# qq456cvb/SLAM-MaskRCNN

Hardware: AMD Instinct MI355X
Metric: Mvoxel-updates/s + frames/s, 512^3 semantic TSDF @ 640x480 (higher is better)
Workload: dtype f32; 1 GPU; C3: 512^3 semantic TSDF integrate (sdf f32, weight i32, colour u8x3, 32-bin u32 instance histogram), synthetic 640x480 depth+RGB+mask stream (seed 1, noise on), frames resident in HBM; frames_cycled=16

## Files before the change

### include/semtsdf.h

```cpp
#ifndef SEMTSDF_H
#define SEMTSDF_H

#include <stddef.h>
#include <stdint.h>

#ifdef __cplusplus
extern "C" {
#endif

#define SEMTSDF_ABI_VERSION 12
#define SEMTSDF_MAX_OBJECTS 32

#define SEMTSDF_OK 0
#define SEMTSDF_ERR_INVALID (-1)
#define SEMTSDF_ERR_HIP (-2)
#define SEMTSDF_ERR_OOM (-3)
#define SEMTSDF_ERR_LABEL (-4)
#define SEMTSDF_ERR_STATE (-5)
#define SEMTSDF_ERR_COMM (-6)
#define SEMTSDF_ERR_UNSUPPORTED (-7)
#define SEMTSDF_NEED_PIXELS 1

#define SEMTSDF_F_SEMANTIC 0x1u
#define SEMTSDF_F_GATE_COLOR 0x2u
// ... 182 lines not shown
typedef struct semtsdf_instance {
    uint64_t voxels;
    uint64_t votes;
    uint64_t support;
    uint64_t sum[3];
    uint64_t rgb_sum[3];
    uint32_t min[3], max[3];
} semtsdf_instance;
int semtsdf_instance_stats(semtsdf_vol* v, float sdf_max, int32_t min_weight,
                           semtsdf_instance out[SEMTSDF_MAX_OBJECTS], uint64_t* overlap );
int semtsdf_remap_instances(semtsdf_vol* v, const uint8_t lut[SEMTSDF_MAX_OBJECTS], int32_t num_objs,
                            void* stream);

int semtsdf_map_words(semtsdf_vol* v, uint64_t* out, uint64_t capacity, uint64_t* count);

int semtsdf_set_instrumentation(semtsdf_vol* v, int enable);
int semtsdf_get_timing(semtsdf_vol* v, semtsdf_timing* out);
int semtsdf_reset_timing(semtsdf_vol* v);

int semtsdf_tsdf_update(float* tsdf_diff, int32_t* tsdf_color, int32_t* tsdf_wt, int32_t* tsdf_cls,
                        int32_t* tsdf_cls_cnt, int vol_dim, const float* vol_start, float voxel,
                        float miu, const float* intrinsic, const uint16_t* depth, const uint8_t* color,
                        const int32_t* cls, const float* extrinsic2init, int width, int height);

#ifdef __cplusplus
}
#endif
#endif
```

### slam-maskrcnn_amd/csrc/semtsdf_api.cpp

```cpp
#include <hip/hip_runtime.h>

#include <algorithm>
#include <cmath>
#include <cstdarg>
#include <cstdio>
#include <cstdlib>
#include <cstring>
#include <mutex>
#include <string>
#include <vector>

#include "../../include/semtsdf.h"
#include "semtsdf_internal.h"

using namespace semtsdf;

namespace {

thread_local std::string g_err;

int fail(int code, const char* fmt, ...) {
    char buf[1024];
    va_list ap;
    va_start(ap, fmt);
// ... 68 lines not shown
    uint8_t* palette_d = nullptr;
    uint8_t* render_d = nullptr;
    float* render_t_d = nullptr;
    unsigned long long* counters_d = nullptr;
    IntegrateRare* rare_d = nullptr;
    float* rcp_table_d = nullptr;
    AssocDecision* decision_h = nullptr;
    void* ray_state_d = nullptr;
    MarchCamera ray_cam{};
    int ray_kind = -1;
    int ray_nrec = 1;
    int ray_next = 0;
    uint32_t n_obs = 0;
    bool maps_dirty = false;
    bool maps_stale = true;
    hipEvent_t maps_ev = nullptr;
    bool maps_ev_set = false;
    hipStream_t map_stream = nullptr;
    bool map_set = false;
    bool multi_stream = false;
    bool color_wide = false;
    int64_t wmax_bound = 0;
    const uint8_t* pending_lut = nullptr;
    unsigned long long* wtrace_d = nullptr;
    unsigned* tile_cost_d = nullptr;
    unsigned* tile_perm_d = nullptr;
    int tile_cap = 0, tile_n = 0;
    bool tables_clean = false;
    unsigned long long votes_dropped_seen = 0;
    int instr = 0;
// ... 9 lines not shown
size_t npx(const semtsdf_vol* v) { return (size_t)v->p.width * (size_t)v->p.height; }

hipStream_t pick(const semtsdf_vol* v, void* s) { return s ? (hipStream_t)s : v->stream; }

int dev_alloc(semtsdf_vol* v, void** p, size_t bytes) {
    if (bytes == 0) { *p = nullptr; return SEMTSDF_OK; }
    hipError_t e = hipMalloc(p, bytes);
    if (e != hipSuccess)
        return fail(e == hipErrorOutOfMemory ? SEMTSDF_ERR_OOM : SEMTSDF_ERR_HIP, "hipMalloc(%zu): %s", bytes,
                    hipGetErrorString(e));
    v->device_bytes += bytes;
    return SEMTSDF_OK;
}

void free_all(semtsdf_vol* v) {
    void* ptrs[] = {v->b.sdf, v->b.wt, v->b.bplain, v->b.boct, v->b.botmp, v->b.bdirty, v->b.dlist, v->b.sflag, v->b.color, v->b.hist, v->b.hmask, v->b.cls, v->b.cls_cnt, v->depth_d, v->rgb_d,
                    v->mask_d, v->cls_d, v->tables_d, v->decision_d,
                    v->num_objs_d, v->probs_d, v->box_d, v->palette_d, v->render_d, v->render_t_d,
                    v->counters_d, v->ray_state_d, v->rcp_table_d, v->wtrace_d, v->exact_d, v->px.bits, v->px.p, v->tile_cost_d, v->tile_perm_d, v->rare_d};
    for (void* q : ptrs)
        if (q) (void)hipFree(q);
    for (auto& f : v->fs)
        for (void* q : {(void*)f.pyr.px, (void*)f.pyr.l0, (void*)f.pyr.l1, (void*)f.unit_list, (void*)f.list_count,
                        (void*)f.units})
            if (q) (void)hipFree(q);
    if (v->decision_h) (void)hipHostFree(v->decision_h);
    for (auto* vec : {&v->ev_integrate, &v->ev_assoc, &v->ev_render, &v->ev_prep})
        for (auto& e : *vec) { (void)hipEventDestroy(e.a); (void)hipEventDestroy(e.b); }
    if (v->maps_ev) (void)hipEventDestroy(v->maps_ev);
    for (auto& f : v->fs) {
        if (f.prep_done) (void)hipEventDestroy(f.prep_done);
// ... 254 lines not shown
            fwrite(h.data(), 8, h.size(), f);
            fclose(f);
        }
    }
    if (ep.a) v->ev_integrate.push_back(ep);
    F.reader = s;
    if (v->async_used && async && own_order) {
        F.free_recorded = false;
    } else if (v->async_used || s != v->stream) {
        if (!F.set_free)
            if (int rc = ensure_prep_stream(v)) return rc;
        HIPC(hipEventRecord(F.set_free, s));
        F.free_recorded = true;
    }
    v->maps_dirty = true;
    v->n_integrate++;
    return SEMTSDF_OK;
}

MarchCamera assoc_camera(const semtsdf_vol* v, const float E[16]) {
    MarchCamera c{};
    const float* Ki = v->p.Kinv;
    c.Kinv[0] = Ki[0]; c.Kinv[1] = Ki[1]; c.Kinv[2] = Ki[2];
    c.Kinv[3] = Ki[4]; c.Kinv[4] = Ki[5]; c.Kinv[5] = Ki[6];
    c.Kinv[6] = Ki[8]; c.Kinv[7] = Ki[9]; c.Kinv[8] = Ki[10];
    for (int i = 0; i < 3; ++i)
        for (int j = 0; j < 3; ++j) c.Rt[i * 3 + j] = E[j * 4 + i];
    for (int i = 0; i < 3; ++i) {
        const double acc = (double)c.Rt[i * 3 + 0] * (double)E[3] + (double)c.Rt[i * 3 + 1] * (double)E[7] +
                           (double)c.Rt[i * 3 + 2] * (double)E[11];
// ... 3 lines not shown
    return c;
}

int order_after_map(semtsdf_vol* v, hipStream_t s) {
    if (!v->map_set || v->map_stream == s) return SEMTSDF_OK;
    v->multi_stream = true;
    if (!v->maps_ev_set) {
        if (!v->maps_ev) HIPC(hipEventCreateWithFlags(&v->maps_ev, order_event_flags()));
        HIPC(hipEventRecord(v->maps_ev, v->map_stream));
        v->maps_ev_set = true;
    }
    HIPC(hipStreamWaitEvent(s, v->maps_ev, 0));
    return SEMTSDF_OK;
}

int ensure_maps(semtsdf_vol* v, hipStream_t s) {
    if (int rc = order_after_map(v, s)) return rc;
    if (!v->maps_dirty && !v->maps_stale) return SEMTSDF_OK;
    HIPC(launch_brick_min(v->g, v->b, v->maps_stale, s));
    v->map_stream = s;
    v->map_set = true;
    v->maps_ev_set = false;
    if (v->multi_stream || s != v->stream) {
        if (!v->maps_ev) HIPC(hipEventCreateWithFlags(&v->maps_ev, order_event_flags()));
        HIPC(hipEventRecord(v->maps_ev, s));
        v->maps_ev_set = true;
    }
    v->maps_dirty = false;
    v->maps_stale = false;
    return SEMTSDF_OK;
}

int after_maps(semtsdf_vol* v, hipStream_t s) { return order_after_map(v, s); }

// ... 350 lines not shown
    const size_t n = g.nvox;
    const size_t px = (size_t)p->width * p->height;
    auto bail = [&](int code) { free_all(v); delete v; return code; };
    int prio_least = 0, prio_greatest = 0;
    if (hipDeviceGetStreamPriorityRange(&prio_least, &prio_greatest) != hipSuccess) prio_greatest = 0;
    if (hipStreamCreateWithPriority(&v->stream, hipStreamNonBlocking, prio_greatest) != hipSuccess)
        return bail(fail(SEMTSDF_ERR_HIP, "hipStreamCreate failed"));
    const bool ci32 = p->flags & SEMTSDF_F_COLOR_I32;
    if ((rc = dev_alloc(v, (void**)&v->b.sdf, n * 4))) return bail(rc);
    if ((rc = dev_alloc(v, (void**)&v->b.wt, n * 4))) return bail(rc);
    if ((rc = dev_alloc(v, (void**)&v->b.sflag, n / 32 + 1))) return bail(rc);
    const size_t nbricks = (size_t)g.nbx * g.nby * g.nbz;
    if ((rc = dev_alloc(v, (void**)&v->b.bplain, nbricks * 4))) return bail(rc);
    if ((rc = dev_alloc(v, (void**)&v->b.boct, nbricks * 8))) return bail(rc);
    if ((rc = dev_alloc(v, (void**)&v->b.botmp, nbricks * 8))) return bail(rc);
    const size_t nquads = (size_t)g.nbx * g.nby * (size_t)((g.nbz + 3) / 4);
    if ((rc = dev_alloc(v, (void**)&v->b.bdirty, nquads * 4))) return bail(rc);
    if ((rc = dev_alloc(v, (void**)&v->b.dlist, (nquads + 1) * 4))) return bail(rc);
    if (nquads && (hipMemset(v->b.bdirty, 0, nquads * 4) != hipSuccess || hipMemset(v->b.dlist, 0, 4) != hipSuccess))
        return bail(fail(SEMTSDF_ERR_HIP, "memset failed"));
    (void)ci32;
    if ((rc = dev_alloc(v, &v->b.color, g.nvox * 4))) return bail(rc);
    if (p->flags & SEMTSDF_F_SEMANTIC)
    {
        if ((rc = dev_alloc(v, (void**)&v->b.hist, g.nvox * kMaxObjects * 4))) return bail(rc);
        if ((rc = dev_alloc(v, (void**)&v->b.hmask, n * 4))) return bail(rc);
    }
    if (p->flags & SEMTSDF_F_VOTE) {
        if ((rc = dev_alloc(v, (void**)&v->b.cls, n * 4))) return bail(rc);
        if ((rc = dev_alloc(v, (void**)&v->b.cls_cnt, n * 4))) return bail(rc);
// ... 964 lines not shown
    }
    v->maps_stale = true;
    HIPC(hipStreamSynchronize(s));
    return SEMTSDF_OK;
}

int semtsdf_map_words(semtsdf_vol* v, uint64_t* out, uint64_t capacity, uint64_t* count) {
    if (!v || !count) return fail(SEMTSDF_ERR_INVALID, "NULL argument");
    HIPC(hipSetDevice(v->device));
    hipStream_t s = v->stream;
    *count = (uint64_t)v->g.nbx * v->g.nby * v->g.nbz;
    if (int rc = ensure_maps(v, s)) return rc;
    const uint64_t n = std::min<uint64_t>(capacity, *count);
    if (out && n) HIPC(hipMemcpyAsync(out, v->b.boct, n * sizeof(uint64_t), hipMemcpyDeviceToHost, s));
    HIPC(hipStreamSynchronize(s));
    return SEMTSDF_OK;
}

int semtsdf_export_surface(semtsdf_vol* v, float sdf_max, int32_t min_weight, semtsdf_surface_point* out,
                           uint64_t capacity, uint64_t* count) {
    static_assert(sizeof(semtsdf_surface_point) == sizeof(SurfacePoint), "surface point layout");
    if (!v || !count) return fail(SEMTSDF_ERR_INVALID, "NULL argument");
    if (!(sdf_max > 0.0f)) return fail(SEMTSDF_ERR_INVALID, "sdf_max must be > 0");
    HIPC(hipSetDevice(v->device));
    hipStream_t s = v->stream;
    if (int rc = after_maps(v, s)) return rc;
    unsigned long long* cnt_d = nullptr;
    HIPC(hipMalloc((void**)&cnt_d, sizeof(unsigned long long)));
    SurfacePoint* pts_d = nullptr;
    auto cleanup = [&]() {
// ... 299 lines not shown
```

### slam-maskrcnn_amd/csrc/semtsdf_internal.h

```cpp
#pragma once
#include <hip/hip_runtime_api.h>
#include <stdint.h>

namespace semtsdf {

constexpr int kMaxObjects = 32;
constexpr int kMaxDetections = 256;
constexpr int kRcpTable = 1024;
constexpr int kZAlign = 32;
#ifndef SEMTSDF_BRICK_DIST_CAP
#define SEMTSDF_BRICK_DIST_CAP 16
#endif
constexpr int kBrickDistCap = SEMTSDF_BRICK_DIST_CAP;
constexpr int kListSegs = 64;
constexpr unsigned kPreWaves = 65534;
constexpr unsigned kFirstTabSlots = kListSegs * 256;
constexpr int kListCountStride = 64;
constexpr int kLists = 3;
constexpr int kListTotalsWord = kLists * kListSegs * kListCountStride;
constexpr int kListCountWords = kListTotalsWord + 8;

struct VolGeom {
    int dimx, dimy, dimz;
    int lz;
// ... 22 lines not shown
struct VolBufs {
    float* sdf;
    int32_t* wt;
    void* color;
    uint32_t* hist;
    uint32_t* hmask;
    int32_t* cls;
    int32_t* cls_cnt;
    float* bplain;
    uint64_t* boct;
    uint64_t* botmp;
    uint32_t* bdirty;
    uint32_t* dlist;
    uint8_t* sflag;
};

struct DepthPyramid {
    uint2* px;
    uint2* l0;
    uint2* l1;
    int w0, h0, w1, h1;
    unsigned rs;
};

__device__ inline unsigned rec_index(const DepthPyramid& p, unsigned u, unsigned v) {
    return __umul24(v >> 2, p.rs) + ((u << 2) | (v & 3u));
}

struct IntegrateRare {
    uint32_t* bdirty;
// ... 174 lines not shown
hipError_t launch_shard_ray_step(const ShardRayArgs& a, hipStream_t s);
hipError_t launch_shard_render_final(const ShardRayArgs& a, hipStream_t s);
hipError_t launch_shard_render_finish(const ShardRayArgs& a, hipStream_t s);
hipError_t launch_shard_assoc_partial(const ShardRayArgs& a, hipStream_t s);
hipError_t launch_shard_assoc_pixels(const ShardRayArgs& a, int32_t* out, hipStream_t s);
hipError_t launch_tables_from_partial(const long long* reduced, AssocTables* t, hipStream_t s);
hipError_t launch_copy_f4(const void* src, void* dst, size_t n16, hipStream_t s);
hipError_t launch_min_i64(long long* dst, const long long* src, size_t n, hipStream_t s);
hipError_t launch_masks_to_labels(const uint8_t* masks, int npx, int n, int min_area, void* scratch, uint8_t* out,
                                  hipStream_t s);
size_t mask_scratch_bytes();
size_t mask_scratch_kept_offset();
hipError_t launch_detections_to_labels(const int32_t* boxes, const void* mini, int dtype, int mh, int mw, int n,
                                       int width, int height, int min_area, void* scratch, uint8_t* out,
                                       uint32_t* areas, hipStream_t s);
hipError_t launch_brick_min(const VolGeom& g, const VolBufs& b, bool all, hipStream_t s);
hipError_t launch_fill_volume(const VolGeom& g, const VolBufs& b, uint32_t flags, hipStream_t s);
hipError_t launch_depth_pyramid(const uint16_t* depth, const uint8_t* rgb, uint8_t* mask, int w, int h,
                                float scale, const DepthPyramid& p, unsigned* list_count, hipStream_t s,
                                const uint8_t* lut = nullptr);
hipError_t launch_vox_chunk(const void* src, void* dst, bool to_ref, const VolGeom& g, uint64_t v0, uint64_t nv,
                            hipStream_t s);
hipError_t launch_color_widen(const uint8_t* narrow, int32_t* wide, uint64_t nvox, hipStream_t s);
hipError_t launch_color_chunk(const void* src, void* dst, bool to_ref, bool ref_i32, bool dev_i32, const VolGeom& g,
                              uint64_t v0, uint64_t nv, hipStream_t s);
hipError_t launch_integrate(const IntegrateArgs& a, hipStream_t s, hipEvent_t e0 = nullptr,
                            hipEvent_t e1 = nullptr);
uint64_t unit_count(const VolGeom& g);
uint64_t unit_list_capacity(const VolGeom& g);
int unit_grid_fits(int dimx, int dimy, int local_z);
hipError_t launch_cull(const IntegrateArgs& a, hipStream_t s);
// ... 62 lines not shown
```

### slam-maskrcnn_amd/csrc/semtsdf_kernels.hip

```cpp
#include <hip/hip_runtime.h>
#include <hip/hip_ext.h>
#include <stdint.h>
#include <limits.h>
#include <stddef.h>
#include <stdlib.h>
#include "semtsdf_internal.h"
#include "semtsdf_libm.h"
#include "semtsdf_steps.h"

namespace semtsdf {

__device__ __forceinline__ int f2i_rd(float x) {
    const float f = floorf(x);
    if (!(f == f)) return 0;
    if (f >= 2147483648.0f) return INT_MAX;
    if (f <= -2147483648.0f) return INT_MIN;
    return (int)f;
}

__device__ __forceinline__ float dot3(float a0, float a1, float a2, float b0, float b1, float b2) {
    return fmaf(a2, b2, fmaf(a1, b1, a0 * b0));
}

typedef float f32x2 __attribute__((ext_vector_type(2)));
// ... 99 lines not shown
}

__global__ __launch_bounds__(256) void k_min_i64(long long* __restrict__ dst, const long long* __restrict__ src, size_t n) {
    for (size_t i = (size_t)blockIdx.x * blockDim.x + threadIdx.x; i < n; i += (size_t)gridDim.x * blockDim.x)
        dst[i] = min(dst[i], src[i]);
}

hipError_t launch_min_i64(long long* dst, const long long* src, size_t n, hipStream_t s) {
    size_t blocks = (n + 255) / 256;
    if (blocks > 4096) blocks = 4096;
    if (blocks == 0) return hipSuccess;
    hipLaunchKernelGGL(k_min_i64, dim3((unsigned)blocks), dim3(256), 0, s, dst, src, n);
    return hipGetLastError();
}

__device__ __forceinline__ void brick_quad_min(const VolGeom& g, const float* __restrict__ sdf,
                                               float* __restrict__ plain, unsigned q, unsigned want) {
    const unsigned nbq = (unsigned)(g.nbz + 3) / 4;
    const int lane = threadIdx.x & 63;
    const int bq = q % nbq, by = (q / nbq) % g.nby, bx = q / (nbq * g.nby);
    const unsigned br0 = ((unsigned)bx * g.nby + (unsigned)by) * g.nbz + (unsigned)bq * 4;
    const int nbr = min(4, g.nbz - bq * 4);
    const int x = bx * 8 + (lane >> 3), y = by * 8 + (lane & 7), z0 = bq * 32;
    float m[4] = {3.0e38f, 3.0e38f, 3.0e38f, 3.0e38f};
    if (x < g.dimx && y < g.dimy) {
        const float* p = sdf + tile_index(g, x, y, z0);
        if (z0 + 32 <= g.lz) {
#pragma unroll
            for (int j = 0; j < 4; ++j) {
                const float4 a = *reinterpret_cast<const float4*>(p + 64 * j);
                const float4 c = *reinterpret_cast<const float4*>(p + 64 * j + 32);
                m[j] = fminf(fminf(fminf(a.x, a.y), fminf(a.z, a.w)), fminf(fminf(c.x, c.y), fminf(c.z, c.w)));
            }
        } else {
            for (int k = 0; k < g.lz - z0; ++k) {
                const float v = p[tile_zterm(k)];
#pragma unroll
                for (int j = 0; j < 4; ++j) m[j] = (k >> 3) == j ? fminf(m[j], v) : m[j];
            }
        }
    }
#pragma unroll
    for (int j = 0; j < 4; ++j)
        for (int off = 32; off > 0; off >>= 1) m[j] = fminf(m[j], __shfl_xor(m[j], off, 64));
    if (lane < nbr && ((want >> lane) & 1u)) {
        const float mj = lane == 0 ? m[0] : lane == 1 ? m[1] : lane == 2 ? m[2] : m[3];
        plain[br0 + lane] = mj;
    }
}

__global__ __launch_bounds__(256) void k_brick_plain(VolGeom g, const float* __restrict__ sdf, float* __restrict__ plain,
                                                     uint32_t* __restrict__ dirty, const uint32_t* __restrict__ dlist,
                                                     int all) {
    const unsigned nbq = (unsigned)(g.nbz + 3) / 4;
    const unsigned nq = (unsigned)g.nbx * g.nby * nbq;
    const unsigned w0 = blockIdx.x * 4 + (threadIdx.x >> 6);
    if (all) {
        if (w0 >= nq) return;
        brick_quad_min(g, sdf, plain, w0, 0xFu);
        if ((threadIdx.x & 63) == 0) dirty[w0] = 0u;
        return;
    }
    const unsigned n = dlist[0];
    for (unsigned i = w0; i < n; i += gridDim.x * 4) {
        const unsigned q = dlist[1 + i];
        const unsigned want = dirty[q];
        brick_quad_min(g, sdf, plain, q, want);
        if ((threadIdx.x & 63) == 0) dirty[q] = 0u;
    }
}

__device__ __forceinline__ float skip_threshold(const VolGeom& g);

__global__ __launch_bounds__(256) void k_brick_dilate(VolGeom g, const float* __restrict__ plain,
                                                      uint64_t* __restrict__ d0, uint32_t* __restrict__ dlist) {
    const unsigned nb = (unsigned)g.nbx * g.nby * g.nbz;
    const unsigned br = blockIdx.x * blockDim.x + threadIdx.x;
    if (br == 0) dlist[0] = 0u;
    if (br >= nb) return;
    const int bz = br % g.nbz, by = (br / g.nbz) % g.nby, bx = br / (g.nbz * g.nby);
    float m = 3.0e38f;
    for (int i = 0; i < 2; ++i)
        for (int j = 0; j < 2; ++j)
            for (int k = 0; k < 2; ++k) {
                const int xx = bx + i, yy = by + j, zz = bz + k;
                if (xx < g.nbx && yy < g.nby && zz < g.nbz) m = fminf(m, plain[((unsigned)xx * g.nby + yy) * g.nbz + zz]);
            }
    d0[br] = m >= skip_threshold(g) ? (uint64_t)kBrickDistCap * 0x0101010101010101ull : 0ull;
}

typedef unsigned short u16x2 __attribute__((ext_vector_type(2)));

template <int AXIS>
__device__ __forceinline__ void oct_unpack(uint64_t wp, uint64_t wn, u16x2 R[4]) {
    const uint32_t pl = (uint32_t)wp, ph = (uint32_t)(wp >> 32), nl = (uint32_t)wn, nh = (uint32_t)(wn >> 32);
    uint32_t r0, r1, r2, r3;
    if (AXIS == 0) {
        r0 = pl & 0x00FF00FFu; r1 = (nl >> 8) & 0x00FF00FFu;
        r2 = ph & 0x00FF00FFu; r3 = (nh >> 8) & 0x00FF00FFu;
    } else if (AXIS == 1) {
        r0 = (pl & 0x000000FFu) | (nl & 0x00FF0000u); r1 = ((pl >> 8) & 0x000000FFu) | ((nl >> 8) & 0x00FF0000u);
        r2 = (ph & 0x000000FFu) | (nh & 0x00FF0000u); r3 = ((ph >> 8) & 0x000000FFu) | ((nh >> 8) & 0x00FF0000u);
    } else {
        r0 = pl & 0x00FF00FFu; r1 = (pl >> 8) & 0x00FF00FFu;
        r2 = nh & 0x00FF00FFu; r3 = (nh >> 8) & 0x00FF00FFu;
    }
    R[0] = __builtin_bit_cast(u16x2, r0); R[1] = __builtin_bit_cast(u16x2, r1);
    R[2] = __builtin_bit_cast(u16x2, r2); R[3] = __builtin_bit_cast(u16x2, r3);
}

template <int AXIS>
__global__ __launch_bounds__(256) void k_brick_oct_axis(VolGeom g, const uint64_t* __restrict__ in,
                                                        uint64_t* __restrict__ out) {
    const unsigned nb = (unsigned)g.nbx * g.nby * g.nbz;
    const unsigned br = blockIdx.x * blockDim.x + threadIdx.x;
    if (br >= nb) return;
    const int bz = br % g.nbz, by = (br / g.nbz) % g.nby, bx = br / (g.nbz * g.nby);
    const int pos = AXIS == 0 ? bx : AXIS == 1 ? by : bz;
    const int n = AXIS == 0 ? g.nbx : AXIS == 1 ? g.nby : g.nbz;
    const int stride = AXIS == 0 ? g.nby * g.nbz : AXIS == 1 ? g.nbz : 1;
    const uint64_t v = in[br];
    u16x2 d[4];
    oct_unpack<0>(v, v, d);
    auto hmax = [](const u16x2* x) {
        const u16x2 m = __builtin_elementwise_max(__builtin_elementwise_max(x[0], x[1]),
                                                  __builtin_elementwise_max(x[2], x[3]));
        return (int)max(m.x, m.y);
    };
    int dmax = hmax(d);
    for (int k0 = 1; k0 < kBrickDistCap && k0 < dmax; k0 += 4) {
        uint64_t wp[4], wn[4];
// ... 3 lines not shown
            wp[i] = (k < kBrickDistCap && pos + k < n) ? in[(int)br + k * stride] : ~0ull;
            wn[i] = (k < kBrickDistCap && pos - k >= 0) ? in[(int)br - k * stride] : ~0ull;
        }
#pragma unroll
        for (int i = 0; i < 4; ++i) {
            u16x2 w[4];
            oct_unpack<AXIS>(wp[i], wn[i], w);
            const u16x2 kk = {(unsigned short)(k0 + i), (unsigned short)(k0 + i)};
#pragma unroll
            for (int j = 0; j < 4; ++j) d[j] = __builtin_elementwise_min(d[j], __builtin_elementwise_max(w[j], kk));
        }
        dmax = hmax(d);
    }
    const uint32_t lo = (uint32_t)d[0].x | ((uint32_t)d[1].x << 8) | ((uint32_t)d[0].y << 16) | ((uint32_t)d[1].y << 24);
    const uint32_t hi = (uint32_t)d[2].x | ((uint32_t)d[3].x << 8) | ((uint32_t)d[2].y << 16) | ((uint32_t)d[3].y << 24);
    out[br] = (uint64_t)lo | ((uint64_t)hi << 32);
}

hipError_t launch_brick_min(const VolGeom& g, const VolBufs& b, bool all, hipStream_t s) {
    const unsigned nb = (unsigned)g.nbx * g.nby * g.nbz;
    if (nb == 0) return hipSuccess;
    const unsigned nq = (unsigned)g.nbx * g.nby * (unsigned)((g.nbz + 3) / 4);
    const unsigned nw = all ? nq : (nq < 4096u ? nq : 4096u);
    hipLaunchKernelGGL(k_brick_plain, dim3((nw + 3) / 4), dim3(256), 0, s, g, b.sdf, b.bplain, b.bdirty, b.dlist,
                       all ? 1 : 0);
    hipLaunchKernelGGL(k_brick_dilate, dim3((nb + 255) / 256), dim3(256), 0, s, g, b.bplain, b.botmp, b.dlist);
    hipLaunchKernelGGL(k_brick_oct_axis<0>, dim3((nb + 255) / 256), dim3(256), 0, s, g, b.botmp, b.boct);
    hipLaunchKernelGGL(k_brick_oct_axis<1>, dim3((nb + 255) / 256), dim3(256), 0, s, g, b.boct, b.botmp);
    hipLaunchKernelGGL(k_brick_oct_axis<2>, dim3((nb + 255) / 256), dim3(256), 0, s, g, b.botmp, b.boct);
    return hipGetLastError();
}

hipError_t launch_fill_volume(const VolGeom& g, const VolBufs& b, uint32_t flags, hipStream_t s) {
    (void)flags;
    const uint64_t n = g.nvox;
    uint64_t blocks = (n / 4 + 255) / 256;
    if (blocks > 8192) blocks = 8192;
    if (blocks == 0) blocks = 1;
    hipLaunchKernelGGL(k_fill_f32, dim3((unsigned)blocks), dim3(256), 0, s, b.sdf, n, g.mu);
    return hipGetLastError();
}

__device__ __forceinline__ void pyramid_tile(const uint16_t* __restrict__ depth, const uint8_t* __restrict__ rgb,
                                             uint8_t* mask, int w, int h, float scale, int vec, const DepthPyramid& p,
// ... 888 lines not shown
template <bool SEM, bool CI32, bool VOTE, bool FREE>
__device__ __forceinline__ void stage_store(const IntegrateArgs& a, const UnitPos& up, unsigned coff,
                                            const StoreMeta& M, const Out& O) {
    const VolGeom& g = a.g;
    const unsigned tmask = M.meta & 15u, gmask = (M.meta >> 4) & 15u, hmode = (M.meta >> 8) & 3u,
                   hlab = M.meta >> 16;
    const bool line = ((__ballot(tmask != 0u) >> ((int)__lane_id() % LZQ + lane_slot((int)__lane_id()) * kUnitLanes)) &
                       kLineLanes) != 0ull;
    if (!line) return;
    const uint64_t v = O.ub + coff;
    {
        const uint64_t cb = __ballot(O.cross);
        const __attribute__((address_space(4))) IntegrateRare* R =
            (const __attribute__((address_space(4))) IntegrateRare*)a.rare;
        if (cb && R->bdirty) {
            const int lane = (int)__lane_id(), j = lane % kUnitLanes;
            const int bz = (up.uz * UZ >> 3) + j;
            const uint64_t pj = ((kLineLanes << (2 * (j & 3))) | (kLineLanes << (2 * (j & 3) + 1)))
                                << (lane_slot(lane) * kUnitLanes);
            if (j < UZ / 8 && (cb & pj) && bz < R->nbz) {
                const unsigned nbq = (unsigned)(R->nbz + 3) >> 2;
                const unsigned q = __umul24(__umul24((unsigned)(up.x * UX >> 3), (unsigned)R->nby) +
                                                (unsigned)(up.uy * UY >> 3), nbq) + ((unsigned)bz >> 2);
                __attribute__((address_space(1))) uint32_t* bd = (__attribute__((address_space(1))) uint32_t*)R->bdirty;
                __attribute__((address_space(1))) uint32_t* dl = (__attribute__((address_space(1))) uint32_t*)R->dlist;
                if (__hip_atomic_fetch_or(bd + q, 1u << (bz & 3), __ATOMIC_RELAXED, __HIP_MEMORY_SCOPE_AGENT) == 0u)
                    dl[1 + __hip_atomic_fetch_add(dl, 1u, __ATOMIC_RELAXED, __HIP_MEMORY_SCOPE_AGENT)] = q;
            }
        }
    }
    if (!(kProbes && a.debug == 10) && tmask != 0u) {
        if (!O.skip) st_state(a.b.sdf + v, O.s4);
        st_state(a.b.wt + v, O.w4);
    }
    {
// ... 2951 lines not shown
```

### slam-maskrcnn_amd/semtsdf/_lib.py

```python
from __future__ import annotations

import ctypes as C
import os

import numpy as np

_HERE = os.path.dirname(os.path.abspath(__file__))
LIB_PATH = os.path.join(_HERE, "libsemtsdf.so")

MAX_OBJECTS = 32

OK = 0
ERR_INVALID = -1
ERR_HIP = -2
ERR_OOM = -3
ERR_LABEL = -4
ERR_STATE = -5
ERR_COMM = -6
ERR_UNSUPPORTED = -7

F_SEMANTIC = 0x1
F_GATE_COLOR = 0x2
F_COLOR_I32 = 0x4
F_VOTE = 0x8
# ... 90 lines not shown
        ("n_integrate", C.c_uint64),
        ("n_assoc", C.c_uint64),
        ("n_render", C.c_uint64),
        ("touched", C.c_uint64),
        ("gated", C.c_uint64),
        ("bricks", C.c_uint64),
        ("prep_ms", C.c_double),
        ("n_prep", C.c_uint64),
        ("free_units", C.c_uint64),
        ("full_units", C.c_uint64),
        ("lazy_voxels", C.c_uint64),
        ("assoc_exact_frames", C.c_uint64),
        ("assoc_exact_rows", C.c_uint64),
        ("touched_lines", C.c_uint64),
        ("assoc_pos_max", C.c_double),
    ]


_P = C.c_void_p
_I = C.c_int
_F = C.c_float
_D = C.c_double
_PP = C.POINTER(C.c_void_p)

SIGNATURES = {
    "semtsdf_last_error": (C.c_char_p, []),
    "semtsdf_abi_version": (_I, []),
    "semtsdf_build_key": (C.c_char_p, []),
    "semtsdf_device_count": (_I, [C.POINTER(C.c_int)]),
    "semtsdf_set_device": (_I, [_I]),
# ... 38 lines not shown
    "semtsdf_shard_note_integrated": (_I, [_P, _P, _P]),
    "semtsdf_min_i64": (_I, [_P, _P, C.c_size_t, _P]),
    "semtsdf_masks_to_labels": (_I, [_P, _I, _I, _I, _I, _P, C.POINTER(C.c_int), _P]),
    "semtsdf_detections_to_labels_workspace": (C.c_size_t, [_I]),
    "semtsdf_detections_to_labels": (_I, [_P, _P, _I, _I, _I, _I, _I, _I, _I, _P, _P, _P, C.POINTER(C.c_int), _P]),
    "semtsdf_copy_bandwidth": (_I, [_I, C.c_size_t, _I, C.POINTER(C.c_double)]),
    "semtsdf_download": (_I, [_P, _P, _P, _P, _P, _P, _P]),
    "semtsdf_download_slab": (_I, [_P, _I, _I, _P, _P, _P, _P, _P, _P]),
    "semtsdf_upload": (_I, [_P, _P, _P, _P, _P, _P, _P]),
    "semtsdf_export_surface": (_I, [_P, _F, C.c_int32, _P, C.c_uint64, C.POINTER(C.c_uint64)]),
    "semtsdf_extract_mesh": (_I, [_P, C.c_int32, _P, C.c_uint64, _P, C.c_uint64, C.POINTER(C.c_uint64),
                                  C.POINTER(C.c_uint64)]),
    "semtsdf_instance_stats": (_I, [_P, _F, C.c_int32, _P, _P]),
    "semtsdf_remap_instances": (_I, [_P, _P, C.c_int32, _P]),
    "semtsdf_map_words": (_I, [_P, _P, C.c_uint64, C.POINTER(C.c_uint64)]),
    "semtsdf_set_instrumentation": (_I, [_P, _I]),
    "semtsdf_get_timing": (_I, [_P, C.POINTER(Timing)]),
    "semtsdf_reset_timing": (_I, [_P]),
    "semtsdf_tsdf_update": (_I, [_P, _P, _P, _P, _P, _I, _P, _F, _F, _P, _P, _P, _P, _P, _I, _I]),
}

_lib = None
_load_error = None


def _bind_torch_runtime():
    if os.environ.get("SEMTSDF_NO_TORCH") == "1":
        return
    try:
        import torch
# ... 53 lines not shown
```

### slam-maskrcnn_amd/semtsdf/volume.py

```python
from __future__ import annotations

import ctypes as C

import numpy as np

from . import _lib as L


def default_params(dim, intrinsics, width, height) -> L.Params:
    lib = L.load()
    p = L.Params()
    intr = L.f32(intrinsics, 4)
    L.check(lib.semtsdf_params_default(C.byref(p), int(dim), L.ptr(intr), int(width), int(height)))
    return p


def place_from_frame(p: L.Params, depth: np.ndarray, mean_depth: float, mode: int) -> L.Params:
    lib = L.load()
    d = np.ascontiguousarray(depth, dtype=np.uint16)
    if d.size != p.width * p.height:
        raise ValueError("depth size does not match params")
    L.check(lib.semtsdf_place_from_frame(C.byref(p), L.ptr(d), float(mean_depth), int(mode)))
    return p

# ... 230 lines not shown
                c(cls, np.int32), c(cls_cnt, np.int32)]
        L.check(L.load().semtsdf_upload(self._h, *[L.ptr(a) for a in arrs]))

    def instance_stats(self, sdf_max: float = 0.2, min_weight: int = 1, overlap: bool = True) -> dict:
        from .instances import instance_stats

        return instance_stats(self, sdf_max, min_weight, overlap)

    def remap_instances(self, lut, num_objs: int = -1, stream=None):
        t = np.ascontiguousarray(np.asarray(lut).reshape(-1))
        if t.size != L.MAX_OBJECTS or (t < 0).any() or (t > 255).any():
            raise ValueError(f"lut must hold {L.MAX_OBJECTS} ids")
        t = t.astype(np.uint8)
        L.check(L.load().semtsdf_remap_instances(self._h, L.ptr(t), int(num_objs), stream))

    def set_instrumentation(self, events: bool = True, count: bool = False, force_exact: bool = False):
        flags = (1 if events else 0) | (2 if count else 0) | (4 if force_exact else 0)
        L.check(L.load().semtsdf_set_instrumentation(self._h, flags))

    def map_words(self):
        import numpy as np
        n = C.c_uint64(0)
        L.check(L.load().semtsdf_map_words(self._h, None, 0, C.byref(n)))
        if n.value == 0:
            return None
        out = np.zeros(n.value, dtype=np.uint64)
        L.check(L.load().semtsdf_map_words(self._h, C.c_void_p(out.ctypes.data), n.value, C.byref(n)))
        return out

    def filter_overlaps_dev(self, probs_ptr: int, box_ptr: int, mask_ptr: int, stream=None) -> L.AssocStats:
        st = L.AssocStats()
        L.check(L.load().semtsdf_filter_overlaps_dev(self._h, C.c_void_p(probs_ptr), C.c_void_p(box_ptr),
                                                     C.c_void_p(mask_ptr), C.byref(st), stream))
        return st

    def timing(self) -> L.Timing:
        t = L.Timing()
        L.check(L.load().semtsdf_get_timing(self._h, C.byref(t)))
        return t

    def reset_timing(self):
        L.check(L.load().semtsdf_reset_timing(self._h))
```

Before: 1.652 million Mvoxel-updates/s.

## Add incremental brick distance-map update driven by flip lists

Adds an incremental mode for the brick skip map: the plain-min pass records bricks whose skip classification flips, then seed and per-axis octahedral distance passes recompute only neighbourhoods of changed bricks using epoch stamps and bounded lists, falling back to full passes on overflow. The aim is to avoid full-volume map rebuilds after each integrate. Separately, the integrate kernel's dirty-brick marking now elects a single lane per crossed brick to cut redundant atomic writes. Adds extra buffers, atomics and a stats API; incremental mode is gated by a brick-count threshold or env/flag.

```diff
diff --git a/include/semtsdf.h b/include/semtsdf.h
--- a/include/semtsdf.h
+++ b/include/semtsdf.h
@@ -220,6 +220,17 @@
 
 int semtsdf_map_words(semtsdf_vol* v, uint64_t* out, uint64_t capacity, uint64_t* count);
 
+typedef struct semtsdf_map_stats {
+    uint32_t incremental;
+    uint32_t dirty_quads;
+    uint32_t plain_flips;
+    uint32_t seed_flips;
+    uint32_t changed[3];
+    uint32_t overflow;
+    uint32_t capacity;
+} semtsdf_map_stats;
+int semtsdf_get_map_stats(semtsdf_vol* v, semtsdf_map_stats* out);
+
 int semtsdf_set_instrumentation(semtsdf_vol* v, int enable);
 int semtsdf_get_timing(semtsdf_vol* v, semtsdf_timing* out);
 int semtsdf_reset_timing(semtsdf_vol* v);
diff --git a/slam-maskrcnn_amd/csrc/semtsdf_api.cpp b/slam-maskrcnn_amd/csrc/semtsdf_api.cpp
--- a/slam-maskrcnn_amd/csrc/semtsdf_api.cpp
+++ b/slam-maskrcnn_amd/csrc/semtsdf_api.cpp
@@ -106,6 +106,10 @@
     uint32_t n_obs = 0;
     bool maps_dirty = false;
     bool maps_stale = true;
+    MapInc mi{};
+    int maps_pending = 0;
+    uint32_t map_epoch = 0;
+    uint32_t map_inc_epoch0 = 0;
     hipEvent_t maps_ev = nullptr;
     bool maps_ev_set = false;
     hipStream_t map_stream = nullptr;
@@ -145,7 +149,7 @@
 }
 
 void free_all(semtsdf_vol* v) {
-    void* ptrs[] = {v->b.sdf, v->b.wt, v->b.bplain, v->b.boct, v->b.botmp, v->b.bdirty, v->b.dlist, v->b.sflag, v->b.color, v->b.hist, v->b.hmask, v->b.cls, v->b.cls_cnt, v->depth_d, v->rgb_d,
+    void* ptrs[] = {v->b.sdf, v->b.wt, v->b.bplain, v->b.boct, v->b.botmp, v->mi.seed, v->mi.octx, v->mi.ctl, v->mi.lists, v->mi.stamp, v->b.bdirty, v->b.dlist, v->b.sflag, v->b.color, v->b.hist, v->b.hmask, v->b.cls, v->b.cls_cnt, v->depth_d, v->rgb_d,
                     v->mask_d, v->cls_d, v->tables_d, v->decision_d,
                     v->num_objs_d, v->probs_d, v->box_d, v->palette_d, v->render_d, v->render_t_d,
                     v->counters_d, v->ray_state_d, v->rcp_table_d, v->wtrace_d, v->exact_d, v->px.bits, v->px.p, v->tile_cost_d, v->tile_perm_d, v->rare_d};
@@ -430,6 +434,7 @@
         F.free_recorded = true;
     }
     v->maps_dirty = true;
+    v->maps_pending++;
     v->n_integrate++;
     return SEMTSDF_OK;
 }
@@ -463,10 +468,31 @@
     return SEMTSDF_OK;
 }
 
+bool maps_incremental(const semtsdf_vol* v) {
+    static const char* env = getenv("SEMTSDF_MAP_INCREMENTAL");
+    if (env && *env) return atoi(env) != 0;
+    if (v->instr & 8) return true;
+    return (uint64_t)v->g.nbx * v->g.nby * v->g.nbz >= kMapIncMinBricks;
+}
+
 int ensure_maps(semtsdf_vol* v, hipStream_t s) {
     if (int rc = order_after_map(v, s)) return rc;
     if (!v->maps_dirty && !v->maps_stale) return SEMTSDF_OK;
-    HIPC(launch_brick_min(v->g, v->b, v->maps_stale, s));
+    uint32_t epoch0 = 0;
+    const bool inc = !v->maps_stale && maps_incremental(v) && v->maps_pending <= kMapIncMaxFrames;
+    v->maps_pending = 0;
+    if (inc) {
+        if (v->map_epoch > 0xFFFFFFF0u) {
+            const size_t nb = (size_t)v->g.nbx * v->g.nby * v->g.nbz;
+            HIPC(hipMemsetAsync(v->mi.stamp, 0, nb * sizeof(uint32_t), s));
+            HIPC(hipMemsetAsync(v->mi.ctl + kMapOvf, 0, kMapLists * sizeof(uint32_t), s));
+            v->map_epoch = 0;
+        }
+        epoch0 = v->map_epoch + 1;
+        v->map_epoch += 4;
+    }
+    HIPC(launch_brick_min(v->g, v->b, v->mi, v->maps_stale ? kMapAll : inc ? kMapIncremental : kMapDirty, epoch0, s));
+    v->map_inc_epoch0 = epoch0;
     v->map_stream = s;
     v->map_set = true;
     v->maps_ev_set = false;
@@ -847,6 +873,15 @@
     if ((rc = dev_alloc(v, (void**)&v->b.bplain, nbricks * 4))) return bail(rc);
     if ((rc = dev_alloc(v, (void**)&v->b.boct, nbricks * 8))) return bail(rc);
     if ((rc = dev_alloc(v, (void**)&v->b.botmp, nbricks * 8))) return bail(rc);
+    if ((rc = dev_alloc(v, (void**)&v->mi.seed, nbricks * 8))) return bail(rc);
+    if ((rc = dev_alloc(v, (void**)&v->mi.octx, nbricks * 8))) return bail(rc);
+    v->mi.cap = map_list_capacity(nbricks);
+    if ((rc = dev_alloc(v, (void**)&v->mi.ctl, kMapCtlWords * 4))) return bail(rc);
+    if ((rc = dev_alloc(v, (void**)&v->mi.lists, (size_t)kMapLists * v->mi.cap * 4))) return bail(rc);
+    if ((rc = dev_alloc(v, (void**)&v->mi.stamp, nbricks * 4))) return bail(rc);
+    if (hipMemset(v->mi.ctl, 0, kMapCtlWords * 4) != hipSuccess ||
+        (nbricks && hipMemset(v->mi.stamp, 0, nbricks * 4) != hipSuccess))
+        return bail(fail(SEMTSDF_ERR_HIP, "memset failed"));
     const size_t nquads = (size_t)g.nbx * g.nby * (size_t)((g.nbz + 3) / 4);
     if ((rc = dev_alloc(v, (void**)&v->b.bdirty, nquads * 4))) return bail(rc);
     if ((rc = dev_alloc(v, (void**)&v->b.dlist, (nquads + 1) * 4))) return bail(rc);
@@ -1841,6 +1876,28 @@
     const uint64_t n = std::min<uint64_t>(capacity, *count);
     if (out && n) HIPC(hipMemcpyAsync(out, v->b.boct, n * sizeof(uint64_t), hipMemcpyDeviceToHost, s));
     HIPC(hipStreamSynchronize(s));
+    return SEMTSDF_OK;
+}
+
+int semtsdf_get_map_stats(semtsdf_vol* v, semtsdf_map_stats* out) {
+    if (!v || !out) return fail(SEMTSDF_ERR_INVALID, "NULL argument");
+    HIPC(hipSetDevice(v->device));
+    *out = semtsdf_map_stats{};
+    out->capacity = v->mi.cap;
+    if (!v->map_set) return SEMTSDF_OK;
+    uint32_t c[kMapCtlWords];
+    HIPC(hipDeviceSynchronize());
+    HIPC(hipMemcpy(c, v->mi.ctl, sizeof(c), hipMemcpyDeviceToHost));
+    if (!v->map_inc_epoch0) return SEMTSDF_OK;
+    out->incremental = 1;
+    out->dirty_quads = c[kMapStatQuads];
+    out->plain_flips = c[kMapStatPlain];
+    out->seed_flips = c[kMapStatSeed];
+    out->changed[0] = c[kMapStatX];
+    out->changed[1] = c[kMapCnt + kMapListXY];
+    out->changed[2] = c[kMapCnt + kMapListXYZ];
+    for (int i = 0; i < kMapLists; ++i)
+        if (c[kMapOvf + i] == v->map_inc_epoch0) out->overflow |= 1u << i;
     return SEMTSDF_OK;
 }
 
diff --git a/slam-maskrcnn_amd/csrc/semtsdf_internal.h b/slam-maskrcnn_amd/csrc/semtsdf_internal.h
--- a/slam-maskrcnn_amd/csrc/semtsdf_internal.h
+++ b/slam-maskrcnn_amd/csrc/semtsdf_internal.h
@@ -60,6 +60,36 @@
     uint32_t* dlist;
     uint8_t* sflag;
 };
+
+constexpr int kMapListPlain = 0;
+constexpr int kMapListSeed = 1;
+constexpr int kMapListX = 2;
+constexpr int kMapListXY = 3;
+constexpr int kMapListXYZ = 4;
+constexpr int kMapLists = 4;
+constexpr int kMapCnt = 0;
+constexpr int kMapOvf = 5;
+constexpr int kMapStatQuads = 9;
+constexpr int kMapStatPlain = 10;
+constexpr int kMapStatSeed = 11;
+constexpr int kMapStatX = 12;
+constexpr int kMapCtlWords = 16;
+constexpr unsigned kMapIncBlocks = 1024;
+constexpr int kMapAll = 0, kMapDirty = 1, kMapIncremental = 2;
+constexpr uint64_t kMapIncMinBricks = 1u << 20;
+constexpr int kMapIncMaxFrames = 4;
+struct MapInc {
+    uint64_t* seed;
+    uint64_t* octx;
+    uint32_t* ctl;
+    uint32_t* lists;
+    uint32_t* stamp;
+    unsigned cap;
+};
+inline unsigned map_list_capacity(uint64_t nbricks) {
+    const uint64_t c = nbricks / 32u;
+    return (unsigned)(c < 256u ? 256u : c);
+}
 
 struct DepthPyramid {
     uint2* px;
@@ -264,7 +294,8 @@
 hipError_t launch_detections_to_labels(const int32_t* boxes, const void* mini, int dtype, int mh, int mw, int n,
                                        int width, int height, int min_area, void* scratch, uint8_t* out,
                                        uint32_t* areas, hipStream_t s);
-hipError_t launch_brick_min(const VolGeom& g, const VolBufs& b, bool all, hipStream_t s);
+hipError_t launch_brick_min(const VolGeom& g, const VolBufs& b, const MapInc& m, int mode, uint32_t epoch0,
+                            hipStream_t s);
 hipError_t launch_fill_volume(const VolGeom& g, const VolBufs& b, uint32_t flags, hipStream_t s);
 hipError_t launch_depth_pyramid(const uint16_t* depth, const uint8_t* rgb, uint8_t* mask, int w, int h,
                                 float scale, const DepthPyramid& p, unsigned* list_count, hipStream_t s,
diff --git a/slam-maskrcnn_amd/csrc/semtsdf_kernels.hip b/slam-maskrcnn_amd/csrc/semtsdf_kernels.hip
--- a/slam-maskrcnn_amd/csrc/semtsdf_kernels.hip
+++ b/slam-maskrcnn_amd/csrc/semtsdf_kernels.hip
@@ -137,8 +137,27 @@
     return hipGetLastError();
 }
 
+__device__ __forceinline__ float skip_threshold(const VolGeom& g);
+
+__device__ __forceinline__ void map_list_append(const MapInc& m, int list, unsigned br, uint32_t epoch0) {
+    const unsigned i = atomicAdd(m.ctl + kMapCnt + list, 1u);
+    if (i < m.cap) m.lists[(size_t)list * m.cap + i] = br;
+    else m.ctl[kMapOvf + list] = epoch0;
+}
+
+__device__ __forceinline__ bool map_lists_full(const MapInc& m, int upto, uint32_t epoch0) {
+    bool f = false;
+    for (int j = 0; j <= upto; ++j) f |= m.ctl[kMapOvf + j] == epoch0;
+    return f;
+}
+
+__device__ __forceinline__ bool map_claim(const MapInc& m, unsigned br, uint32_t epoch) {
+    return atomicExch(m.stamp + br, epoch) != epoch;
+}
+
 __device__ __forceinline__ void brick_quad_min(const VolGeom& g, const float* __restrict__ sdf,
-                                               float* __restrict__ plain, unsigned q, unsigned want) {
+                                               float* __restrict__ plain, unsigned q, unsigned want, bool flips,
+                                               const MapInc& mi, uint32_t epoch0) {
     const unsigned nbq = (unsigned)(g.nbz + 3) / 4;
     const int lane = threadIdx.x & 63;
     const int bq = q % nbq, by = (q / nbq) % g.nby, bx = q / (nbq * g.nby);
@@ -168,19 +187,27 @@
         for (int off = 32; off > 0; off >>= 1) m[j] = fminf(m[j], __shfl_xor(m[j], off, 64));
     if (lane < nbr && ((want >> lane) & 1u)) {
         const float mj = lane == 0 ? m[0] : lane == 1 ? m[1] : lane == 2 ? m[2] : m[3];
+        if (flips) {
+            const float thr = skip_threshold(g);
+            if ((plain[br0 + lane] >= thr) != (mj >= thr)) map_list_append(mi, kMapListPlain, br0 + lane, epoch0);
+        }
         plain[br0 + lane] = mj;
     }
 }
 
 __global__ __launch_bounds__(256) void k_brick_plain(VolGeom g, const float* __restrict__ sdf, float* __restrict__ plain,
                                                      uint32_t* __restrict__ dirty, const uint32_t* __restrict__ dlist,
-                                                     int all) {
+                                                     int all, int flips, MapInc mi, uint32_t epoch0) {
     const unsigned nbq = (unsigned)(g.nbz + 3) / 4;
     const unsigned nq = (unsigned)g.nbx * g.nby * nbq;
     const unsigned w0 = blockIdx.x * 4 + (threadIdx.x >> 6);
+    if (blockIdx.x == 0 && threadIdx.x == 0) {
+        mi.ctl[kMapCnt + kMapListXY] = 0u;
+        mi.ctl[kMapCnt + kMapListXYZ] = 0u;
+    }
     if (all) {
         if (w0 >= nq) return;
-        brick_quad_min(g, sdf, plain, w0, 0xFu);
+        brick_quad_min(g, sdf, plain, w0, 0xFu, false, mi, epoch0);
         if ((threadIdx.x & 63) == 0) dirty[w0] = 0u;
         return;
     }
@@ -188,19 +215,12 @@
     for (unsigned i = w0; i < n; i += gridDim.x * 4) {
         const unsigned q = dlist[1 + i];
         const unsigned want = dirty[q];
-        brick_quad_min(g, sdf, plain, q, want);
+        brick_quad_min(g, sdf, plain, q, want, flips != 0, mi, epoch0);
         if ((threadIdx.x & 63) == 0) dirty[q] = 0u;
     }
 }
 
-__device__ __forceinline__ float skip_threshold(const VolGeom& g);
-
-__global__ __launch_bounds__(256) void k_brick_dilate(VolGeom g, const float* __restrict__ plain,
-                                                      uint64_t* __restrict__ d0, uint32_t* __restrict__ dlist) {
-    const unsigned nb = (unsigned)g.nbx * g.nby * g.nbz;
-    const unsigned br = blockIdx.x * blockDim.x + threadIdx.x;
-    if (br == 0) dlist[0] = 0u;
-    if (br >= nb) return;
+__device__ __forceinline__ uint64_t brick_seed_word(const VolGeom& g, const float* __restrict__ plain, unsigned br) {
     const int bz = br % g.nbz, by = (br / g.nbz) % g.nby, bx = br / (g.nbz * g.nby);
     float m = 3.0e38f;
     for (int i = 0; i < 2; ++i)
@@ -209,7 +229,46 @@
                 const int xx = bx + i, yy = by + j, zz = bz + k;
                 if (xx < g.nbx && yy < g.nby && zz < g.nbz) m = fminf(m, plain[((unsigned)xx * g.nby + yy) * g.nbz + zz]);
             }
-    d0[br] = m >= skip_threshold(g) ? (uint64_t)kBrickDistCap * 0x0101010101010101ull : 0ull;
+    return m >= skip_threshold(g) ? (uint64_t)kBrickDistCap * 0x0101010101010101ull : 0ull;
+}
+
+__global__ __launch_bounds__(256) void k_brick_dilate(VolGeom g, const float* __restrict__ plain,
+                                                      uint64_t* __restrict__ d0, uint32_t* __restrict__ dlist) {
+    const unsigned nb = (unsigned)g.nbx * g.nby * g.nbz;
+    const unsigned br = blockIdx.x * blockDim.x + threadIdx.x;
+    if (br == 0) dlist[0] = 0u;
+    if (br >= nb) return;
+    d0[br] = brick_seed_word(g, plain, br);
+}
+
+__global__ __launch_bounds__(256) void k_brick_seed_inc(VolGeom g, const float* __restrict__ plain, MapInc mi,
+                                                        uint32_t* __restrict__ dlist, uint32_t epoch0) {
+    const unsigned nb = (unsigned)g.nbx * g.nby * g.nbz;
+    const unsigned t = blockIdx.x * blockDim.x + threadIdx.x, nt = gridDim.x * blockDim.x;
+    const unsigned n = mi.ctl[kMapCnt + kMapListPlain];
+    if (t == 0) {
+        mi.ctl[kMapStatQuads] = dlist[0];
+        dlist[0] = 0u;
+        mi.ctl[kMapStatPlain] = n;
+    }
+    if (map_lists_full(mi, kMapListPlain, epoch0)) {
+        for (unsigned br = t; br < nb; br += nt) mi.seed[br] = brick_seed_word(g, plain, br);
+        return;
+    }
+    for (unsigned i = t; i < n * 8u; i += nt) {
+        const unsigned e = mi.lists[(size_t)kMapListPlain * mi.cap + (i >> 3)];
+        const int bz = (int)(e % g.nbz) - (int)(i & 1u), by = (int)((e / g.nbz) % g.nby) - (int)((i >> 1) & 1u),
+                  bx = (int)(e / (g.nbz * g.nby)) - (int)((i >> 2) & 1u);
+        if (bx < 0 || by < 0 || bz < 0) continue;
+        const unsigned br = ((unsigned)bx * g.nby + (unsigned)by) * g.nbz + (unsigned)bz;
+        const bool own = map_claim(mi, br, epoch0);
+        const uint64_t old = mi.seed[br];
+        const uint64_t w = brick_seed_word(g, plain, br);
+        if (own && old != w) {
+            mi.seed[br] = w;
+            map_list_append(mi, kMapListSeed, br, epoch0);
+        }
+    }
 }
 
 typedef unsigned short u16x2 __attribute__((ext_vector_type(2)));
@@ -233,11 +292,7 @@
 }
 
 template <int AXIS>
-__global__ __launch_bounds__(256) void k_brick_oct_axis(VolGeom g, const uint64_t* __restrict__ in,
-                                                        uint64_t* __restrict__ out) {
-    const unsigned nb = (unsigned)g.nbx * g.nby * g.nbz;
-    const unsigned br = blockIdx.x * blockDim.x + threadIdx.x;
-    if (br >= nb) return;
+__device__ __forceinline__ uint64_t brick_oct_axis_word(const VolGeom& g, const uint64_t* __restrict__ in, unsigned br) {
     const int bz = br % g.nbz, by = (br / g.nbz) % g.nby, bx = br / (g.nbz * g.nby);
     const int pos = AXIS == 0 ? bx : AXIS == 1 ? by : bz;
     const int n = AXIS == 0 ? g.nbx : AXIS == 1 ? g.nby : g.nbz;
@@ -271,20 +326,74 @@
     }
     const uint32_t lo = (uint32_t)d[0].x | ((uint32_t)d[1].x << 8) | ((uint32_t)d[0].y << 16) | ((uint32_t)d[1].y << 24);
     const uint32_t hi = (uint32_t)d[2].x | ((uint32_t)d[3].x << 8) | ((uint32_t)d[2].y << 16) | ((uint32_t)d[3].y << 24);
-    out[br] = (uint64_t)lo | ((uint64_t)hi << 32);
-}
-
-hipError_t launch_brick_min(const VolGeom& g, const VolBufs& b, bool all, hipStream_t s) {
+    return (uint64_t)lo | ((uint64_t)hi << 32);
+}
+
+template <int AXIS>
+__global__ __launch_bounds__(256) void k_brick_oct_axis(VolGeom g, const uint64_t* __restrict__ in,
+                                                        uint64_t* __restrict__ out) {
+    const unsigned nb = (unsigned)g.nbx * g.nby * g.nbz;
+    const unsigned br = blockIdx.x * blockDim.x + threadIdx.x;
+    if (br >= nb) return;
+    out[br] = brick_oct_axis_word<AXIS>(g, in, br);
+}
+
+template <int AXIS>
+__global__ __launch_bounds__(256) void k_brick_oct_axis_inc(VolGeom g, const uint64_t* __restrict__ in,
+                                                            uint64_t* __restrict__ out, MapInc mi, uint32_t epoch0) {
+    constexpr int kIn = kMapListSeed + AXIS, kOut = kIn + 1;
+    constexpr unsigned kWin = 2u * kBrickDistCap - 1u;
+    const unsigned nb = (unsigned)g.nbx * g.nby * g.nbz;
+    const unsigned t = blockIdx.x * blockDim.x + threadIdx.x, nt = gridDim.x * blockDim.x;
+    const unsigned n = mi.ctl[kMapCnt + kIn];
+    if (t == 0) {
+        if (AXIS < 2) mi.ctl[kMapStatSeed + AXIS] = n;
+        mi.ctl[kMapCnt + kIn - 1] = 0u;
+    }
+    if (map_lists_full(mi, kIn, epoch0)) {
+        for (unsigned br = t; br < nb; br += nt) out[br] = brick_oct_axis_word<AXIS>(g, in, br);
+        return;
+    }
+    const int na = AXIS == 0 ? g.nbx : AXIS == 1 ? g.nby : g.nbz;
+    const int stride = AXIS == 0 ? g.nby * g.nbz : AXIS == 1 ? g.nbz : 1;
+    for (unsigned i = t; i < n * kWin; i += nt) {
+        const unsigned e = mi.lists[(size_t)kIn * mi.cap + i / kWin];
+        const int off = (int)(i % kWin) - (kBrickDistCap - 1);
+        const int pos = AXIS == 0 ? (int)(e / (g.nbz * g.nby)) : AXIS == 1 ? (int)((e / g.nbz) % g.nby) : (int)(e % g.nbz);
+        if (pos + off < 0 || pos + off >= na) continue;
+        const unsigned br = (unsigned)((int)e + off * stride);
+        const bool own = map_claim(mi, br, epoch0 + 1u + AXIS);
+        const uint64_t old = out[br];
+        const uint64_t w = brick_oct_axis_word<AXIS>(g, in, br);
+        if (own && old != w) {
+            out[br] = w;
+            if (AXIS < 2) map_list_append(mi, kOut, br, epoch0);
+            else atomicAdd(mi.ctl + kMapCnt + kOut, 1u);
+        }
+    }
+}
+
+hipError_t launch_brick_min(const VolGeom& g, const VolBufs& b, const MapInc& m, int mode, uint32_t epoch0,
+                            hipStream_t s) {
     const unsigned nb = (unsigned)g.nbx * g.nby * g.nbz;
     if (nb == 0) return hipSuccess;
+    const bool all = mode == kMapAll;
     const unsigned nq = (unsigned)g.nbx * g.nby * (unsigned)((g.nbz + 3) / 4);
     const unsigned nw = all ? nq : (nq < 4096u ? nq : 4096u);
     hipLaunchKernelGGL(k_brick_plain, dim3((nw + 3) / 4), dim3(256), 0, s, g, b.sdf, b.bplain, b.bdirty, b.dlist,
-                       all ? 1 : 0);
-    hipLaunchKernelGGL(k_brick_dilate, dim3((nb + 255) / 256), dim3(256), 0, s, g, b.bplain, b.botmp, b.dlist);
-    hipLaunchKernelGGL(k_brick_oct_axis<0>, dim3((nb + 255) / 256), dim3(256), 0, s, g, b.botmp, b.boct);
-    hipLaunchKernelGGL(k_brick_oct_axis<1>, dim3((nb + 255) / 256), dim3(256), 0, s, g, b.boct, b.botmp);
-    hipLaunchKernelGGL(k_brick_oct_axis<2>, dim3((nb + 255) / 256), dim3(256), 0, s, g, b.botmp, b.boct);
+                       all ? 1 : 0, mode == kMapIncremental ? 1 : 0, m, epoch0);
+    if (mode != kMapIncremental) {
+        hipLaunchKernelGGL(k_brick_dilate, dim3((nb + 255) / 256), dim3(256), 0, s, g, b.bplain, m.seed, b.dlist);
+        hipLaunchKernelGGL(k_brick_oct_axis<0>, dim3((nb + 255) / 256), dim3(256), 0, s, g, m.seed, m.octx);
+        hipLaunchKernelGGL(k_brick_oct_axis<1>, dim3((nb + 255) / 256), dim3(256), 0, s, g, m.octx, b.botmp);
+        hipLaunchKernelGGL(k_brick_oct_axis<2>, dim3((nb + 255) / 256), dim3(256), 0, s, g, b.botmp, b.boct);
+        return hipGetLastError();
+    }
+    const unsigned ng = (nb + 255) / 256 < kMapIncBlocks ? (nb + 255) / 256 : kMapIncBlocks;
+    hipLaunchKernelGGL(k_brick_seed_inc, dim3(ng), dim3(256), 0, s, g, b.bplain, m, b.dlist, epoch0);
+    hipLaunchKernelGGL(k_brick_oct_axis_inc<0>, dim3(ng), dim3(256), 0, s, g, m.seed, m.octx, m, epoch0);
+    hipLaunchKernelGGL(k_brick_oct_axis_inc<1>, dim3(ng), dim3(256), 0, s, g, m.octx, b.botmp, m, epoch0);
+    hipLaunchKernelGGL(k_brick_oct_axis_inc<2>, dim3(ng), dim3(256), 0, s, g, b.botmp, b.boct, m, epoch0);
     return hipGetLastError();
 }
 
@@ -1203,11 +1312,13 @@
         const __attribute__((address_space(4))) IntegrateRare* R =
             (const __attribute__((address_space(4))) IntegrateRare*)a.rare;
         if (cb && R->bdirty) {
-            const int lane = (int)__lane_id(), j = lane % kUnitLanes;
+            const int lane = (int)__lane_id(), j = lane_zq(lane) >> 1;
             const int bz = (up.uz * UZ >> 3) + j;
-            const uint64_t pj = ((kLineLanes << (2 * (j & 3))) | (kLineLanes << (2 * (j & 3) + 1)))
-                                << (lane_slot(lane) * kUnitLanes);
-            if (j < UZ / 8 && (cb & pj) && bz < R->nbz) {
+            const uint64_t pj = ((kLineLanes << (2 * j)) | (kLineLanes << (2 * j + 1))) << (lane_slot(lane) * kUnitLanes);
+            const uint64_t mine = cb & pj;
+            const unsigned below = __builtin_amdgcn_mbcnt_hi((uint32_t)(mine >> 32), __builtin_amdgcn_mbcnt_lo((uint32_t)mine, 0u));
+            const bool crossed = (((lane & 32) ? (uint32_t)(cb >> 32) : (uint32_t)cb) >> (lane & 31)) & 1u;
+            if (crossed && below == 0u && bz < R->nbz) {
                 const unsigned nbq = (unsigned)(R->nbz + 3) >> 2;
                 const unsigned q = __umul24(__umul24((unsigned)(up.x * UX >> 3), (unsigned)R->nby) +
                                                 (unsigned)(up.uy * UY >> 3), nbq) + ((unsigned)bz >> 2);
diff --git a/slam-maskrcnn_amd/semtsdf/_lib.py b/slam-maskrcnn_amd/semtsdf/_lib.py
--- a/slam-maskrcnn_amd/semtsdf/_lib.py
+++ b/slam-maskrcnn_amd/semtsdf/_lib.py
@@ -128,6 +128,18 @@
         ("assoc_exact_rows", C.c_uint64),
         ("touched_lines", C.c_uint64),
         ("assoc_pos_max", C.c_double),
+    ]
+
+
+class MapStats(C.Structure):
+    _fields_ = [
+        ("incremental", C.c_uint32),
+        ("dirty_quads", C.c_uint32),
+        ("plain_flips", C.c_uint32),
+        ("seed_flips", C.c_uint32),
+        ("changed", C.c_uint32 * 3),
+        ("overflow", C.c_uint32),
+        ("capacity", C.c_uint32),
     ]
 
 
@@ -196,6 +208,7 @@
     "semtsdf_instance_stats": (_I, [_P, _F, C.c_int32, _P, _P]),
     "semtsdf_remap_instances": (_I, [_P, _P, C.c_int32, _P]),
     "semtsdf_map_words": (_I, [_P, _P, C.c_uint64, C.POINTER(C.c_uint64)]),
+    "semtsdf_get_map_stats": (_I, [_P, C.POINTER(MapStats)]),
     "semtsdf_set_instrumentation": (_I, [_P, _I]),
     "semtsdf_get_timing": (_I, [_P, C.POINTER(Timing)]),
     "semtsdf_reset_timing": (_I, [_P]),
diff --git a/slam-maskrcnn_amd/semtsdf/volume.py b/slam-maskrcnn_amd/semtsdf/volume.py
--- a/slam-maskrcnn_amd/semtsdf/volume.py
+++ b/slam-maskrcnn_amd/semtsdf/volume.py
@@ -268,8 +268,9 @@
         t = t.astype(np.uint8)
         L.check(L.load().semtsdf_remap_instances(self._h, L.ptr(t), int(num_objs), stream))
 
-    def set_instrumentation(self, events: bool = True, count: bool = False, force_exact: bool = False):
-        flags = (1 if events else 0) | (2 if count else 0) | (4 if force_exact else 0)
+    def set_instrumentation(self, events: bool = True, count: bool = False, force_exact: bool = False,
+                            incremental_maps: bool = False):
+        flags = (1 if events else 0) | (2 if count else 0) | (4 if force_exact else 0) | (8 if incremental_maps else 0)
         L.check(L.load().semtsdf_set_instrumentation(self._h, flags))
 
     def map_words(self):
@@ -282,6 +283,11 @@
         L.check(L.load().semtsdf_map_words(self._h, C.c_void_p(out.ctypes.data), n.value, C.byref(n)))
         return out
 
+    def map_stats(self) -> L.MapStats:
+        st = L.MapStats()
+        L.check(L.load().semtsdf_get_map_stats(self._h, C.byref(st)))
+        return st
+
     def filter_overlaps_dev(self, probs_ptr: int, box_ptr: int, mask_ptr: int, stream=None) -> L.AssocStats:
         st = L.AssocStats()
         L.check(L.load().semtsdf_filter_overlaps_dev(self._h, C.c_void_p(probs_ptr), C.c_void_p(box_ptr),
```

Measured after the change: 1.586 million Mvoxel-updates/s. -4.0%, worse.
